# qradiolink/qradiolink

Measured on AMD Instinct MI355X. Metric: IQ MSamples/sec through RX demod chain, higher is better.
Workload: dtype f32

## Files before the change

### include/qrl_hip.h

```cpp
#ifndef QRL_HIP_H
#define QRL_HIP_H
#include <stddef.h>
#include <stdint.h>

#ifdef __cplusplus
extern "C" {
#endif

typedef enum {
    QRL_OK = 0,
    QRL_ERR_ARG = -1,
    QRL_ERR_NO_DEVICE = -2,
    QRL_ERR_HIP = -3,
    QRL_ERR_NOMEM = -4,
    QRL_ERR_TOO_BIG = -5,
    QRL_ERR_STATE = -6
} qrl_status;

enum {
    QRL_MODEM_BPSK2K = 0, QRL_MODEM_QPSK20K = 1, QRL_MODEM_QPSKVIDEO = 2, QRL_MODEM_4FSK2K = 3, QRL_MODEM_4FSK10KFM = 4, QRL_MODEM_4FSK2KFM = 5, QRL_MODEM_4FSK1KFM = 6, QRL_MODEM_QPSK2K = 7,
    QRL_MODEM_NBFM2500 = 8, QRL_MODEM_NBFM5000 = 9, QRL_MODEM_WBFM = 10, QRL_MODEM_USB2500 = 11, QRL_MODEM_LSB2500 = 12, QRL_MODEM_CW600USB = 13 , QRL_MODEM_AM5000 = 14,
    QRL_MODEM_2FSK2KFM = 15, QRL_MODEM_2FSK1KFM = 16, QRL_MODEM_2FSK2K = 17, QRL_MODEM_2FSK1K = 18,
    QRL_MODEM_2FSK10KFM = 19, QRL_MODEM_GMSK2K = 20, QRL_MODEM_GMSK1K = 21, QRL_MODEM_GMSK10K = 22,
    QRL_MODEM_BPSK1K = 24, QRL_MODEM_BPSK8 = 25 , QRL_MODEM_QPSK250K = 26, QRL_MODEM_4FSK100K = 27, QRL_MODEM_M17 = 40, QRL_MODEM_DMR = 41
// ... 18 lines not shown
    size_t max_chunk;
    void* hip_stream;
    int enable_side_outputs;
    int time_domain_samp_rate;
    double time_domain_filter_width;
} qrl_demod_config;

typedef struct {
    float* filtered;      size_t filtered_cap;
    float* constellation; size_t constellation_cap;
    uint8_t* bits_a;      size_t bits_cap;
    uint8_t* bits_b;
    uint32_t* counts;
    float* audio;         size_t audio_cap;
} qrl_demod_out;

int qrl_demod_create(qrl_ctx* ctx, const qrl_demod_config* cfg, qrl_demod** out);
void qrl_demod_destroy(qrl_demod* d);
int qrl_demod_reset(qrl_demod* d);
int qrl_demod_set_carrier_offset(qrl_demod* d, double carrier_offset_hz);
int qrl_demod_set_carrier_offsets(qrl_demod* d, const double* hz);
#define QRL_DMO_RECORD_BYTES 40
int qrl_demod_set_dmo_output(qrl_demod* d, uint8_t* frames, size_t cap_frames, uint32_t* counts);
enum { QRL_OPT_OVERLAP = 1, QRL_OPT_UNFUSED_DEC2 = 2, QRL_OPT_FLL_SLIM = 3 , QRL_OPT_GROUPED = 4, QRL_OPT_INPUT_RESIDENT = 5 };
int qrl_demod_set_option(qrl_demod* d, int option, int value);
int qrl_demod_out_caps(const qrl_demod* d, size_t n, size_t* filtered_cap, size_t* constellation_cap, size_t* bits_cap);
int qrl_demod_audio_cap(const qrl_demod* d, size_t n, size_t* audio_cap);
int qrl_demod_set_squelch(qrl_demod* d, double db);
int qrl_demod_time_domain_cap(const qrl_demod* d, size_t n, size_t* cap);
int qrl_demod_set_time_domain_output(qrl_demod* d, float* samples, size_t cap, uint32_t* counts);
int qrl_demod_set_ctcss(qrl_demod* d, float tone_hz);
int qrl_demod_set_agc(qrl_demod* d, float attack, float decay);
int qrl_demod_set_filter_width(qrl_demod* d, int filter_width);
int qrl_demod_set_gain(qrl_demod* d, float value);

int qrl_demod_process(qrl_demod* d, const float* iq, size_t stride, size_t n, const qrl_demod_out* out);
int qrl_demod_sync(qrl_demod* d);
void* qrl_demod_stream(qrl_demod* d);
int qrl_demod_internal_streams(qrl_demod* d, void* out[3]);
int qrl_demod_stream_wait(qrl_demod* d, void* hip_stream);

int qrl_demod_profile(qrl_demod* d, int enable);
int qrl_demod_profile_read(qrl_demod* d, double* kernel_ms, uint64_t* launches, const char** kernel_name);

int qrl_demod_process_host(qrl_demod* d, const float* iq_host, size_t stride, size_t n,
                           uint8_t* bits_a_host, uint8_t* bits_b_host, size_t bits_cap, uint32_t* counts_host);

// ... 170 lines not shown
```

### qradiolink_amd/__init__.py

```python
import ctypes as C
import os

import numpy as np

_HERE = os.path.dirname(os.path.abspath(__file__))
LIB_PATH = os.environ.get("QRL_LIB_PATH") or os.path.join(_HERE, "libqrl_hip.so")

MODEM_2FSK2KFM, MODEM_2FSK1KFM, MODEM_2FSK2K, MODEM_2FSK1K, MODEM_2FSK10KFM = 15, 16, 17, 18, 19
MODEM_GMSK2K, MODEM_GMSK1K, MODEM_GMSK10K = 20, 21, 22
MODEM_QPSK250K = 26
MODEM_QPSK20K, MODEM_QPSKVIDEO, MODEM_QPSK2K = 1, 2, 7
MODEM_BPSK2K, MODEM_BPSK1K = 0, 24
MODEM_4FSK2K, MODEM_4FSK10KFM, MODEM_4FSK2KFM, MODEM_4FSK1KFM, MODEM_4FSK100K = 3, 4, 5, 6, 27
MODEM_BPSK8 = 25
MODEM_NBFM2500, MODEM_NBFM5000, MODEM_WBFM, MODEM_AM5000 = 8, 9, 10, 14
MODEM_USB2500, MODEM_LSB2500, MODEM_CW600USB = 11, 12, 13
MODEM_M17 = 40
MODEM_DMR = 41
OPT_OVERLAP, OPT_UNFUSED_DEC2, OPT_FLL_SLIM, OPT_GROUPED, OPT_INPUT_RESIDENT = 1, 2, 3, 4, 5
CHAN_OPT_LEGACY_PFB, CHAN_OPT_LEGACY_TAIL, CHAN_OPT_SERIAL_TAIL = 1, 2, 3
WIN_HAMMING, WIN_HANN, WIN_BLACKMAN, WIN_RECTANGULAR, WIN_BLACKMAN_HARRIS = 0, 1, 2, 3, 5


class QrlError(RuntimeError):
    pass


class _Config(C.Structure):
    _fields_ = [("modem_type", C.c_int), ("use_mode_defaults", C.c_int), ("sps", C.c_int), ("samp_rate", C.c_int),
                ("carrier_freq", C.c_int), ("filter_width", C.c_int), ("fm", C.c_int), ("device_samp_rate", C.c_int),
                ("carrier_offset_hz", C.c_double), ("batch", C.c_int), ("max_chunk", C.c_size_t),
                ("hip_stream", C.c_void_p), ("enable_side_outputs", C.c_int), ("time_domain_samp_rate", C.c_int), ("time_domain_filter_width", C.c_double)]


class _ModConfig(C.Structure):
    _fields_ = [("modem_type", C.c_int), ("use_mode_defaults", C.c_int), ("sps", C.c_int), ("samp_rate", C.c_int),
                ("carrier_freq", C.c_int), ("filter_width", C.c_int), ("fm", C.c_int), ("batch", C.c_int),
                ("max_bytes", C.c_size_t), ("hip_stream", C.c_void_p), ("bb_gain", C.c_float),
                ("device_samp_rate", C.c_int), ("carrier_offset_hz", C.c_double)]


class _ChanConfig(C.Structure):
# ... 900 lines not shown
```

### qradiolink_amd/csrc/devmath.hpp

```cpp
#pragma once
#include <hip/hip_runtime.h>
#include <stdint.h>
#include "../../include/qrl_contracts.h"

namespace qrl {

__device__ __forceinline__ float poly_sin(float x)
{
    const float z = x * x;
    float p = fmaf(z, -1.9515295891e-4f, 8.3321608736e-3f);
    p = fmaf(z, p, -1.6666654611e-1f);
    return fmaf(x * z, p, x);
}
__device__ __forceinline__ float poly_cos(float x)
{
    const float z = x * x;
    float p = fmaf(z, 2.443315711809948e-5f, -1.388731625493765e-3f);
    p = fmaf(z, p, 4.166664568298827e-2f);
    const float q = fmaf(z, -0.5f, 1.0f);
    return fmaf(z * z, p, q);
}
__device__ __forceinline__ float2 quad_fix(int q, float ps, float pc)
{
    const bool swap = q & 1;
    const uint32_t c0 = __float_as_uint(swap ? ps : pc), s0 = __float_as_uint(swap ? pc : ps);
    const uint32_t negc = ((uint32_t)(q + 1) & 2u) << 30, negs = ((uint32_t)q & 2u) << 30;
    return make_float2(__uint_as_float(c0 ^ negc), __uint_as_float(s0 ^ negs));
}
// ... 103 lines not shown
```

### qradiolink_amd/csrc/engine.cpp

```cpp
#include "host_common.hpp"
#include "firdes.hpp"
#include <algorithm>
#include <cmath>
#include <complex>
#include <cstdio>
#include <cstdlib>
#include <cstring>
#include <memory>
#include <new>
#include <string>
#include <mutex>
#include <set>
#include <vector>

using namespace qrl;

static thread_local std::string g_last_error;
int qrl_set_error(int code, const std::string& msg) { g_last_error = msg; return code; }

namespace qrl {
static thread_local bool t_launch_error = false;
hipError_t dyn_lds_limit(const void* kernel, int bytes)
{
    static std::mutex mu;
// ... 177 lines not shown
    }
};

}

struct qrl_demod {
    qrl_ctx* ctx = nullptr;
    qrl_demod_config cfg{};
    hipStream_t stream = nullptr;
    bool own_stream = false;
    hipStream_t tail = nullptr;
    hipStream_t fecs = nullptr;
    hipEvent_t ev_q[2] = {nullptr, nullptr}, ev_fec[2] = {nullptr, nullptr}; bool q_valid[2] = {false, false};
    bool grouped = false, grouped_capable = false, fec_deferred = false; FecParams fec_pending{}; int fec_pending_slot = 0;
    DevBuf<uint64_t> qp_snap;
    hipEvent_t ev_ff = nullptr, ev_tail = nullptr;
    hipStream_t pre = nullptr; hipEvent_t ev_pre = nullptr, ev_fe[2] = {nullptr, nullptr}; bool fe_valid[2] = {false, false}; bool pre_pending = false;
    bool input_resident = false;
    hipEvent_t ev_user[4] = {nullptr, nullptr, nullptr, nullptr};
    bool tail_pending = false;
    bool qpsk_fll = false, fsk4_disc = false;
    bool m17 = false;
    DevBuf<float2> s2g, disc4_taps; DevBuf<float> sym4_taps; int disc4_nt = 0, sym4_nt = 0;
    bool fll_slim = false;
    bool d2f_capable = false, d2f = false; DevBuf<float> d2f_taps;
    bool overlap = false, overlap_capable = false; hipEvent_t ev_tail2[2] = {nullptr, nullptr}; bool tail2_valid[2] = {false, false}; uint64_t call_no = 0;
    enum Family { F_2FSK, F_GMSK, F_QPSK, F_DMR, F_4FSK, F_BPSK, F_DSSS, F_ANALOG } fam = F_2FSK;
    int branches = 2;

    int fe_decim = 1, interp = 1, decim = 1, target = 0, sps_eff = 0;
    bool fm = false;

    DecimStage fe;
    DecimStage first;
    DecimStage scope; DevBuf<float2> s_scope; uint32_t scope_mask = 0; uint64_t n_scope = 0; int scope_D = 10;
    float2* scope_out = nullptr; size_t scope_cap = 0; uint32_t* scope_counts = nullptr;
    DevBuf<float> rs_taps; int rs_Jp = 0;
    DevBuf<float> filt_taps; int filt_nt = 0;
    DevBuf<float> symf_taps; int symf_nt = 0;
    DevBuf<float2> disc_up, disc_lo; int disc_nt = 0;
    DevBuf<float> ff_tf, ff_ts; DevBuf<float2> ff_up, ff_lo;
    DevBuf<float2> fll_lo, fll_up; float fll_alpha = 0, fll_beta = 0, fll_maxf = 0;
    DevBuf<float> atan_tab, mmse_tab;
    float demod_gain = 0;
    float ss_alpha = 0, ss_beta = 0, ss_maxp = 0, ss_minp = 0;

// ... 535 lines not shown
        if (use_pre) {
            if (fe_valid[slot ^ 1]) HIPCHK(hipStreamWaitEvent(pre, ev_fe[slot ^ 1], 0));
            launch_hist_save(h, B, pre);
            HIPCHK(hipEventRecord(ev_pre, pre));
            pre_pending = true;
        } else launch_hist_save(h, B, stream);
        hist_flip = !hist_flip;
    }
    if (overlap) {
        HIPCHK(hipEventRecord(ev_ff, stream));
        HIPCHK(hipStreamWaitEvent(tail, ev_ff, 0));
        HIPCHK(hipMemsetAsync(counts, 0, (size_t)B * 4 * sizeof(uint32_t), tail));
    }
    const uint32_t c2 = (uint32_t)(n2_1 - n2_0);
    const bool side = cfg.enable_side_outputs && out;
    if (fam == F_DSSS || fam == F_ANALOG) {
        if (int rr = fam == F_DSSS ? dsss_stages(n2_0, n2_1, out, counts, side) : analog_stages(n2_0, n2_1, out, counts, side)) return rr;
        HIPCHK(hipGetLastError());
        if (take_launch_error()) return QRL_ERR_HIP;
        n_in = n_in1; n1 = n1_1; n2 = n2_1; ++call_no;
        return QRL_OK;
    }
    RingC filt_in = r2;
    if (fam == F_2FSK || fam == F_BPSK || (fam == F_QPSK && qpsk_fll)) {
        FllParams f{};
        f.in = r2; f.out = r2l; f.q0 = n2_0; f.count = c2; f.st = fll_st.p;
        f.lower = fll_lo.p; f.upper = fll_up.p; f.nt = fam == F_2FSK ? 16 : 32; f.alpha = fll_alpha; f.beta = fll_beta; f.max_freq = fll_maxf;
        f.slim = fll_slim ? 1 : 0;
        if (!(QRL_DEV_SKIP & 1)) launch_fll(f, B, cs);
        filt_in = r2l;
    }
    const bool fused_2fsk = fam == F_2FSK && !fm && filt_nt <= 41 && disc_nt <= 41 && symf_nt <= 25;
    if (fam == F_DMR) {
        RingC dem_in = r2;
        if (m17) {
            FirCcfParams f{};
            f.in = r2; f.out = r2f; f.q0 = n2_0; f.count = c2; f.taps = filt_taps.p; f.nt = filt_nt;
            f.port = side && out->filtered ? reinterpret_cast<float2*>(out->filtered) : nullptr;
            f.port_cap = side ? out->filtered_cap : 0;
            f.counts = counts;
            launch_fir_ccf(f, B, cs);
            dem_in = r2f;
        }
        QuadDemodParams q{}; q.in = dem_in; q.out = r2d; q.q0 = n2_0; q.count = c2; q.gain = demod_gain; q.atan_tab = atan_tab.p;
        launch_quad_demod(q, B, cs);
        if (!overlap && tail_pending) { HIPCHK(hipStreamWaitEvent(stream, ev_tail, 0)); tail_pending = false; }
        FirFffParams f{}; f.in = r2d; f.out = r3; f.q0 = n2_0; f.count = c2; f.taps = symf_taps.p; f.nt = symf_nt;
        launch_fir_fff(f, B, cs);
        if (!overlap) { HIPCHK(hipEventRecord(ev_ff, stream)); HIPCHK(hipStreamWaitEvent(tail, ev_ff, 0)); }
    } else if (fused_2fsk) {
        if (!overlap && tail_pending) { HIPCHK(hipStreamWaitEvent(stream, ev_tail, 0)); tail_pending = false; }
        Fsk2FfParams f{};
        f.in = filt_in; f.out = r3; f.q0 = n2_0; f.count = c2;
        f.tf = ff_tf.p; f.nf = fsk2_ff_padded(filt_nt); f.up = ff_up.p; f.lo = ff_lo.p; f.nb = fsk2_ff_padded(disc_nt);
        f.ts = ff_ts.p; f.ns = fsk2_ff_padded(symf_nt);
        f.port = side && out->filtered ? reinterpret_cast<float2*>(out->filtered) : nullptr;
        f.port_cap = side ? out->filtered_cap : 0;
        f.counts = counts;
        if (!(QRL_DEV_SKIP & 2)) launch_2fsk_ff(f, B, cs);
        if (!overlap) { HIPCHK(hipEventRecord(ev_ff, stream)); HIPCHK(hipStreamWaitEvent(tail, ev_ff, 0)); }
    } else {
        if (!d2f) {
            FirCcfParams f{};
            f.in = filt_in; f.out = r2f; f.q0 = n2_0; f.count = c2; f.taps = filt_taps.p; f.nt = filt_nt;
            f.port = side && out->filtered ? reinterpret_cast<float2*>(out->filtered) : nullptr;
            f.port_cap = side ? out->filtered_cap : 0;
            f.counts = counts;
            launch_fir_ccf(f, B, cs);
        }
        if (fam == F_QPSK || fam == F_BPSK) {
        } else if (fsk4_disc) {
            RingC r2l4{s2l.p, s2_mask}, r2g{s2g.p, s2_mask};
            Disc4fskParams d{}; d.in = r2f; d.out = r2l4; d.q0 = n2_0; d.count = c2; d.taps = disc4_taps.p; d.nt = disc4_nt;
            launch_disc_4fsk(d, B, cs);
            FirCcfParams f{}; f.in = r2l4; f.out = r2g; f.q0 = n2_0; f.count = c2; f.taps = sym4_taps.p; f.nt = sym4_nt;
            launch_fir_ccf(f, B, cs);
        } else if (fam == F_GMSK || fam == F_4FSK || fm) {
            QuadDemodParams q{}; q.in = r2f; q.out = r2d; q.q0 = n2_0; q.count = c2; q.gain = demod_gain; q.atan_tab = atan_tab.p;
            launch_quad_demod(q, B, cs);
        } else {
            Disc2fskParams d{}; d.in = r2f; d.out = r2d; d.q0 = n2_0; d.count = c2; d.up = disc_up.p; d.lo = disc_lo.p; d.nt = disc_nt;
            launch_disc_2fsk(d, B, cs);
// ... 383 lines not shown
        if (int rs = d->sync_all()) return rs;
        if ((r = d->dmo_st.alloc(d->cfg.batch)) || (r = d->dmo_golay.upload(golay1987_table()))) return r;
        std::vector<DmoState> ds(d->cfg.batch);
        for (auto& x : ds) { std::memset(&x, 0, sizeof x); x.endPtr = 9999; }
        if (hipMemcpy(d->dmo_st.p, ds.data(), ds.size() * sizeof(DmoState), hipMemcpyHostToDevice) != hipSuccess) return QRL_ERR_HIP;
    }
    d->dmo_out = frames; d->dmo_cap = (uint32_t)cap_frames; d->dmo_counts = counts;
    return QRL_OK;
}
int qrl_demod_set_option(qrl_demod* d, int option, int value)
{
    if (!d) return QRL_ERR_ARG;
    switch (option) {
    case QRL_OPT_OVERLAP:
        if (value != 0 && !d->overlap_capable) return qrl_set_error(QRL_ERR_ARG, "overlapped mode exists for the 2FSK family only");
        if (int rs = d->sync_all()) return rs;
        d->overlap = value != 0;
        d->tail2_valid[0] = d->tail2_valid[1] = false;
        return QRL_OK;
    case QRL_OPT_FLL_SLIM:
        if (int rs = d->sync_all()) return rs;
        d->fll_slim = value != 0;
        return QRL_OK;
    case QRL_OPT_GROUPED:
        if (value != 0 && !d->grouped_capable) return qrl_set_error(QRL_ERR_ARG, "the grouped order exists for the gr_demod_qpsk chain only");
        if (int rs = d->sync_all()) return rs;
        d->grouped = value != 0;
        return QRL_OK;
    case QRL_OPT_INPUT_RESIDENT: {
        if (int rs = d->sync_all()) return rs;
        if (value != 0 && d->pre) {
            DecimStage& st = d->fe.used ? d->fe : d->first;
            if (st.edge_len && !st.edge_b.p) if (int r = st.edge_b.alloc((size_t)d->cfg.batch * st.edge_len)) return qrl_set_error(r, "edge scratch");
        }
        d->input_resident = value != 0;
        return QRL_OK;
    }
    case QRL_OPT_UNFUSED_DEC2:
        if (!d->d2f_capable) return qrl_set_error(QRL_ERR_ARG, "this chain has no fused 1:2 decimator + shaping filter");
        if (d->n_in != 0) return qrl_set_error(QRL_ERR_STATE, "QRL_OPT_UNFUSED_DEC2 can only be set before the first sample (the two forms carry different state)");
        d->d2f = value == 0;
        return QRL_OK;
    default:
        return qrl_set_error(QRL_ERR_ARG, "unknown option");
    }
}
// ... 221 lines not shown
```

### qradiolink_amd/csrc/engine.hpp

```cpp
#pragma once
#include <hip/hip_runtime.h>
#include <stdint.h>
#include <vector>

namespace qrl {

hipError_t dyn_lds_limit(const void* kernel, int bytes);
bool take_launch_error();

int create_role_stream(hipStream_t* s, int priority, const char* role);

struct RingC { float2* p; uint32_t mask; };
struct RingF { float* p; uint32_t mask; };
struct RingB { uint8_t* p; uint32_t mask; };

template <class Pp>
__device__ __forceinline__ void rot_select(Pp& c, const Pp& p, uint32_t b)
{
    c = p; c.rot_acc = p.rot_acc_s[b]; c.rot_inc = p.rot_inc_s[b]; c.rot_lo = p.rot_lo + (size_t)b * 512;
}
#define ROT_VIEW(T, PS, P, SRC, B) T P##_ps_; if constexpr (PS) rot_select(P##_ps_, SRC, (uint32_t)(B)); const T& P = (PS) ? P##_ps_ : SRC
std::vector<float2> rot_fine_table(uint64_t inc);
void launch_rot_ps_advance(uint64_t* acc, const uint64_t* inc, int B, uint64_t delta, hipStream_t s);
void launch_rot_ps_fill(uint64_t* acc, uint64_t* inc, float2* lo, int B, int set_acc, uint64_t acc0, uint64_t inc0, const float2* lo0, hipStream_t s);
// ... 72 lines not shown
                      float2* port; size_t port_cap; uint32_t* counts; };
struct FirFffParams { RingF in; RingF out; uint64_t q0; uint32_t count; const float* taps; int nt; };
struct QuadDemodParams { RingC in; RingF out; uint64_t q0; uint32_t count; float gain; const float* atan_tab;
                         RingF out2; float gain2;
                         int16_t* s16; size_t s16_cap; float s16_level, s16_scale; uint32_t* s16_counts; };
struct Disc2fskParams { RingC in; RingF out; uint64_t q0; uint32_t count; const float2* up; const float2* lo; int nt; };
struct Disc4fskParams { RingC in; RingC out; uint64_t q0; uint32_t count; const float2* taps; int nt; };
void launch_disc_4fsk(const Disc4fskParams& p, int batch, hipStream_t s);
struct Fsk2FfParams { RingC in; RingF out; uint64_t q0; uint32_t count;
                      const float* tf; int nf; const float2* up; const float2* lo; int nb; const float* ts; int ns;
                      float2* port; size_t port_cap; uint32_t* counts; };
void launch_2fsk_ff(const Fsk2FfParams& p, int batch, hipStream_t s);
int fsk2_ff_padded(int n);
void launch_fir_ccf(const FirCcfParams& p, int batch, hipStream_t s);
void launch_fir_fff(const FirFffParams& p, int batch, hipStream_t s);
void launch_quad_demod(const QuadDemodParams& p, int batch, hipStream_t s);
void launch_disc_2fsk(const Disc2fskParams& p, int batch, hipStream_t s);

struct FllState { float phase, freq; float2 dl[32]; };
struct FllParams { RingC in; RingC out; uint64_t q0; uint32_t count; FllState* st;
                   const float2* lower; const float2* upper; int nt; float alpha, beta, max_freq;
                   int slim; };
void launch_fll(const FllParams& p, int batch, hipStream_t s);

struct SymSyncState { uint64_t ii; uint64_t oo; float mu, avg, inst; float x0, x1, x2, d0, d1, d2; };
struct SymSyncParams {
    RingF in; uint64_t avail;
    RingB soft;
    SymSyncState* st;
    const float* mmse;
    float alpha, beta, maxp, minp;
    int ted; float soft_mul, soft_add;
    int slicer;
    float tail_scale;
    int tail;
    uint8_t* bits; size_t bits_cap;
    float2* port; size_t port_cap; uint32_t* counts;
    int slim;
};
void launch_symsync_ff(const SymSyncParams& p, int batch, hipStream_t s);

struct QpskState {
    uint64_t ii, oo;
    float gain;
    float c1_phase, c1_freq;
    float mu, avg, inst;
// ... 202 lines not shown
```

### qradiolink_amd/csrc/kernels_ff.hip

```cpp
#include "devmath.hpp"
#include "engine.hpp"
#include <cstdlib>

namespace qrl {

__device__ __forceinline__ float2 ringc_at(const RingC& r, int b, int64_t i)
{
    if (i < 0) return make_float2(0.f, 0.f);
    return r.p[(size_t)b * (r.mask + 1u) + ((uint32_t)i & r.mask)];
}
__device__ __forceinline__ float ringf_at(const RingF& r, int b, int64_t i)
{
    if (i < 0) return 0.f;
    return r.p[(size_t)b * (r.mask + 1u) + ((uint32_t)i & r.mask)];
}

__global__ __launch_bounds__(256) void k_fir_ccf(const FirCcfParams P)
{
    const int b = blockIdx.y;
    const uint32_t t = blockIdx.x * 256u + threadIdx.x;
    if (t >= P.count) return;
    if (t == 0 && P.counts) P.counts[b * 4 + 0] = P.count;
    const int64_t n = (int64_t)(P.q0 + t);
    float ar = 0.f, ai = 0.f;
// ... 172 lines not shown
    const float m3 = sqrtf(re[2] * re[2] + im[2] * im[2]), m4 = sqrtf(re[3] * re[3] + im[3] * im[3]);
    const float A = 0.707107f;
    float2 v = make_float2(0.f, 0.f);
    if (m1 > m2 && m1 > m3 && m1 > m4) v = make_float2(-A, -A);
    else if (m2 > m1 && m2 > m3 && m2 > m4) v = make_float2(-A, A);
    else if (m3 > m2 && m3 > m1 && m3 > m4) v = make_float2(A, A);
    else if (m4 > m2 && m4 > m1 && m4 > m3) v = make_float2(A, -A);
    P.out.p[(size_t)b * (P.out.mask + 1u) + ((uint32_t)n & P.out.mask)] = v;
}
void launch_disc_4fsk(const Disc4fskParams& p, int batch, hipStream_t s)
{
    if (!p.count) return;
    hipLaunchKernelGGL(k_disc_4fsk, dim3((p.count + 255) / 256, batch), dim3(256), 0, s, p);
}

void launch_disc_2fsk(const Disc2fskParams& p, int batch, hipStream_t s)
{
    if (!p.count) return;
    hipLaunchKernelGGL(k_disc_2fsk, dim3((p.count + 255) / 256, batch), dim3(256), 0, s, p);
}

constexpr int FF_PL = 280, FF_PF = 264, FF_PD = 264;

template <int PITCH, int NQ, typename TapT, typename ItemT, typename Fma>
__device__ __forceinline__ void ff_window4(const ItemT* __restrict__ tile, int w, int nq_rt, const TapT* __restrict__ taps, Fma&& fma4)
{
    ItemT cur[4], nxt[4];
#pragma unroll
    for (int s = 0; s < 4; ++s) cur[s] = tile[s * PITCH + w];
    auto quad = [&](int q) {
        --w;
#pragma unroll
        for (int s = 0; s < 4; ++s) nxt[s] = tile[s * PITCH + w];
        const TapT h0 = taps[4 * q], h1 = taps[4 * q + 1], h2 = taps[4 * q + 2], h3 = taps[4 * q + 3];
        fma4(h0, cur[0], cur[1], cur[2], cur[3]);
        fma4(h1, nxt[3], cur[0], cur[1], cur[2]);
        fma4(h2, nxt[2], nxt[3], cur[0], cur[1]);
        fma4(h3, nxt[1], nxt[2], nxt[3], cur[0]);
#pragma unroll
        for (int s = 0; s < 4; ++s) cur[s] = nxt[s];
    };
    if constexpr (NQ > 0) {
#pragma unroll 4
        for (int q = 0; q < NQ; ++q) quad(q);
    } else {
        for (int q = 0; q < nq_rt; ++q) quad(q);
    }
}

template <int NQF, int NQB, int NQS>
__global__ __launch_bounds__(256) void k_2fsk_ff(const Fsk2FfParams P)
{
    __shared__ float2 lt[4 * FF_PL];
    __shared__ float2 ft[4 * FF_PF];
    __shared__ float dt[4 * FF_PD];
    const int b = blockIdx.y, tid = threadIdx.x;
    const int hf = P.nf - 1, hb = P.nb - 1, hs = P.ns - 1;
    const int T = 1024 - hb - hs;
    const int64_t n0t = (int64_t)P.q0 + (int64_t)blockIdx.x * T;
    const int nl = 1024 + hf, nd = T + hs;
    if (tid < 4) { lt[tid * FF_PL] = make_float2(0.f, 0.f); ft[tid * FF_PF] = make_float2(0.f, 0.f); dt[tid * FF_PD] = 0.f; }
    {
        float2 v[5];
#pragma unroll
        for (int it = 0; it < 5; ++it) {
            const int64_t a = n0t - (hf + hb + hs) + tid + 256 * it;
            v[it] = P.in.p[(size_t)b * (P.in.mask + 1u) + ((uint32_t)a & P.in.mask)];
            if (a < 0) v[it] = make_float2(0.f, 0.f);
        }
#pragma unroll
        for (int it = 0; it < 5; ++it) {
            const int i = tid + 256 * it;
            if (i < nl) lt[(i & 3) * FF_PL + (i >> 2) + 1] = v[it];
        }
    }
    __syncthreads();
    {
        float2 a[4] = {{0.f, 0.f}, {0.f, 0.f}, {0.f, 0.f}, {0.f, 0.f}};
        ff_window4<FF_PL, NQF>(lt, tid + (hf >> 2) + 1, (hf >> 2) + 1, P.tf,
                          [&](float h, const float2& x0, const float2& x1, const float2& x2, const float2& x3) {
                              a[0].x = fmaf(h, x0.x, a[0].x); a[0].y = fmaf(h, x0.y, a[0].y);
                              a[1].x = fmaf(h, x1.x, a[1].x); a[1].y = fmaf(h, x1.y, a[1].y);
                              a[2].x = fmaf(h, x2.x, a[2].x); a[2].y = fmaf(h, x2.y, a[2].y);
                              a[3].x = fmaf(h, x3.x, a[3].x); a[3].y = fmaf(h, x3.y, a[3].y);
                          });
#pragma unroll
        for (int r = 0; r < 4; ++r) {
            const bool neg = n0t - (hb + hs) + 4 * tid + r < 0;
            ft[r * FF_PF + tid + 1] = neg ? make_float2(0.f, 0.f) : a[r];
        }
    }
    __syncthreads();
    if (4 * tid < nd) {
        float ar[4] = {0.f, 0.f, 0.f, 0.f}, ai[4] = {0.f, 0.f, 0.f, 0.f}, br[4] = {0.f, 0.f, 0.f, 0.f}, bi[4] = {0.f, 0.f, 0.f, 0.f};
        const int nq = NQB > 0 ? NQB : (hb >> 2) + 1;
        int w = tid + (hb >> 2) + 1;
        float2 cur[4], nxt[4];
#pragma unroll
        for (int s = 0; s < 4; ++s) cur[s] = ft[s * FF_PF + w];
        auto step = [&](const float2 h, const float2& x0, const float2& x1, const float2& x2, const float2& x3) {
// ... 13 lines not shown
            step(P.up[4 * q + 2], nxt[2], nxt[3], cur[0], cur[1]);
            step(P.up[4 * q + 3], nxt[1], nxt[2], nxt[3], cur[0]);
#pragma unroll
            for (int s = 0; s < 4; ++s) cur[s] = nxt[s];
        };
        if constexpr (NQB > 0) {
#pragma unroll 4
            for (int q = 0; q < NQB; ++q) quad(q);
        } else {
            for (int q = 0; q < nq; ++q) quad(q);
        }
#pragma unroll
        for (int r = 0; r < 4; ++r) {
            const float ur = ar[r] - bi[r], ui = ai[r] + br[r], lr = ar[r] + bi[r], li = ai[r] - br[r];
            const float mu = sqrtf(ur * ur + ui * ui);
            const float ml = sqrtf(lr * lr + li * li);
            float v = mu / ml;
            if (!(v >= 0.0f)) v = 0.0f;
            if (v > 2.0f) v = 2.0f;
            dt[r * FF_PD + tid + 1] = (n0t - hs + 4 * tid + r < 0) ? 0.f : v + (-1.0f);
        }
    }
    __syncthreads();
    if (4 * tid < T) {
        float a[4] = {0.f, 0.f, 0.f, 0.f};
        ff_window4<FF_PD, NQS>(dt, tid + (hs >> 2) + 1, (hs >> 2) + 1, P.ts,
                          [&](float h, float x0, float x1, float x2, float x3) {
                              a[0] = fmaf(h, x0, a[0]); a[1] = fmaf(h, x1, a[1]); a[2] = fmaf(h, x2, a[2]); a[3] = fmaf(h, x3, a[3]);
                          });
        const uint32_t t0 = blockIdx.x * (uint32_t)T + 4u * tid;
        if (t0 == 0 && P.counts) P.counts[b * 4 + 0] = P.count;
        const int wf = tid + ((hb + hs) >> 2) + 1;
#pragma unroll
        for (int r = 0; r < 4; ++r) {
            const uint32_t t = t0 + r;
            if (t < P.count) {
                const int64_t n = n0t + 4 * tid + r;
                P.out.p[(size_t)b * (P.out.mask + 1u) + ((uint32_t)n & P.out.mask)] = a[r];
                if (P.port && t < P.port_cap) P.port[(size_t)b * P.port_cap + t] = ft[r * FF_PF + wf];
            }
        }
    }
}
int fsk2_ff_padded(int n) { return (n - 1 + 3) / 4 * 4 + 1; }
void launch_2fsk_ff(const Fsk2FfParams& p, int batch, hipStream_t s)
{
    if (!p.count) return;
// ... 10 lines not shown
```

### qradiolink_amd/csrc/kernels_loops.hip

```cpp
#include "devmath.hpp"
#include "engine.hpp"

namespace qrl {


#ifndef QRL_FLL_CH
#define QRL_FLL_CH 32
#endif
#ifndef QRL_FLL_TH
#define QRL_FLL_TH 256
#endif
template <int CTRL> __device__ __forceinline__ float dpp_quad(float v)
{
    return __builtin_bit_cast(float, __builtin_amdgcn_mov_dpp(__builtin_bit_cast(int, v), CTRL, 0xF, 0xF, true));
}

template <int NT, int FLL_TH, int FLL_CH>
__global__ __launch_bounds__(FLL_TH) void k_fll(const FllParams P, int batch)
{
    constexpr int FLL_NS = FLL_TH / 4;
    constexpr int GL = NT / 4;
    __shared__ float2 win[FLL_NS][FLL_CH + 1];
    __shared__ float2 tl[NT], tu[NT];
    __shared__ float2 dump[FLL_TH];
    const int tid = threadIdx.x;
    const int sl = tid >> 2, g = tid & 3;
    const int b0 = blockIdx.x * FLL_NS;
    const int b = b0 + sl;
    const bool active = b < batch;
    for (int k = tid; k < NT; k += FLL_TH) { tl[k] = P.lower[k]; tu[k] = P.upper[k]; }
    float phase = 0.f, freq = 0.f;
    float2 dl[GL];
    if (active) {
        const FllState& s = P.st[b];
        phase = s.phase; freq = s.freq;
#pragma unroll
        for (int t = 0; t < GL; ++t) dl[t] = s.dl[g * GL + t];
    } else {
// ... 358 lines not shown
```

Baseline: 531,300.

## Fuse 2FSK FLL loop with feed-forward filter chain in one warp-specialized kernel

Adds a kernel where one set of wavefronts runs the serial FLL band-edge loop per stream while other wavefronts run the 2FSK FIR/discriminator/symbol-filter chain on the previous window, with the default option turning it on. This avoids the separate FLL kernel writing its output to a global ring and the FF kernel reading it back, and overlaps the latency-bound serial loop with the filter arithmetic. The standalone FF kernel also skips work past the valid count in the last block. The fused path adds prologue recomputation of lookahead windows and extra LDS, and it may lower occupancy.

Measured after the change: 507,400. -4.5%, worse.

```diff
diff --git a/include/qrl_hip.h b/include/qrl_hip.h
--- a/include/qrl_hip.h
+++ b/include/qrl_hip.h
@@ -64,7 +64,8 @@
 int qrl_demod_set_carrier_offsets(qrl_demod* d, const double* hz);
 #define QRL_DMO_RECORD_BYTES 40
 int qrl_demod_set_dmo_output(qrl_demod* d, uint8_t* frames, size_t cap_frames, uint32_t* counts);
-enum { QRL_OPT_OVERLAP = 1, QRL_OPT_UNFUSED_DEC2 = 2, QRL_OPT_FLL_SLIM = 3 , QRL_OPT_GROUPED = 4, QRL_OPT_INPUT_RESIDENT = 5 };
+enum { QRL_OPT_OVERLAP = 1, QRL_OPT_UNFUSED_DEC2 = 2, QRL_OPT_FLL_SLIM = 3 , QRL_OPT_GROUPED = 4, QRL_OPT_INPUT_RESIDENT = 5,
+       QRL_OPT_FUSED_FLL_FF = 6  };
 int qrl_demod_set_option(qrl_demod* d, int option, int value);
 int qrl_demod_out_caps(const qrl_demod* d, size_t n, size_t* filtered_cap, size_t* constellation_cap, size_t* bits_cap);
 int qrl_demod_audio_cap(const qrl_demod* d, size_t n, size_t* audio_cap);
diff --git a/qradiolink_amd/__init__.py b/qradiolink_amd/__init__.py
--- a/qradiolink_amd/__init__.py
+++ b/qradiolink_amd/__init__.py
@@ -17,7 +17,7 @@
 MODEM_USB2500, MODEM_LSB2500, MODEM_CW600USB = 11, 12, 13
 MODEM_M17 = 40
 MODEM_DMR = 41
-OPT_OVERLAP, OPT_UNFUSED_DEC2, OPT_FLL_SLIM, OPT_GROUPED, OPT_INPUT_RESIDENT = 1, 2, 3, 4, 5
+OPT_OVERLAP, OPT_UNFUSED_DEC2, OPT_FLL_SLIM, OPT_GROUPED, OPT_INPUT_RESIDENT, OPT_FUSED_FLL_FF = 1, 2, 3, 4, 5, 6
 CHAN_OPT_LEGACY_PFB, CHAN_OPT_LEGACY_TAIL, CHAN_OPT_SERIAL_TAIL = 1, 2, 3
 WIN_HAMMING, WIN_HANN, WIN_BLACKMAN, WIN_RECTANGULAR, WIN_BLACKMAN_HARRIS = 0, 1, 2, 3, 5
 
diff --git a/qradiolink_amd/csrc/devmath.hpp b/qradiolink_amd/csrc/devmath.hpp
--- a/qradiolink_amd/csrc/devmath.hpp
+++ b/qradiolink_amd/csrc/devmath.hpp
@@ -4,6 +4,11 @@
 #include "../../include/qrl_contracts.h"
 
 namespace qrl {
+
+template <int CTRL> __device__ __forceinline__ float dpp_quad(float v)
+{
+    return __builtin_bit_cast(float, __builtin_amdgcn_mov_dpp(__builtin_bit_cast(int, v), CTRL, 0xF, 0xF, true));
+}
 
 __device__ __forceinline__ float poly_sin(float x)
 {
diff --git a/qradiolink_amd/csrc/engine.cpp b/qradiolink_amd/csrc/engine.cpp
--- a/qradiolink_amd/csrc/engine.cpp
+++ b/qradiolink_amd/csrc/engine.cpp
@@ -223,6 +223,7 @@
     bool qpsk_fll = false, fsk4_disc = false;
     bool m17 = false;
     DevBuf<float2> s2g, disc4_taps; DevBuf<float> sym4_taps; int disc4_nt = 0, sym4_nt = 0;
+    int fused_fll_ff = 1;
     bool fll_slim = false;
     bool d2f_capable = false, d2f = false; DevBuf<float> d2f_taps;
     bool overlap = false, overlap_capable = false; hipEvent_t ev_tail2[2] = {nullptr, nullptr}; bool tail2_valid[2] = {false, false}; uint64_t call_no = 0;
@@ -804,15 +805,19 @@
         return QRL_OK;
     }
     RingC filt_in = r2;
+    const bool fused_2fsk = fam == F_2FSK && !fm && filt_nt <= 41 && disc_nt <= 41 && symf_nt <= 25;
+    FllFfParams fl{};
+    bool fused_fll = false;
     if (fam == F_2FSK || fam == F_BPSK || (fam == F_QPSK && qpsk_fll)) {
         FllParams f{};
         f.in = r2; f.out = r2l; f.q0 = n2_0; f.count = c2; f.st = fll_st.p;
         f.lower = fll_lo.p; f.upper = fll_up.p; f.nt = fam == F_2FSK ? 16 : 32; f.alpha = fll_alpha; f.beta = fll_beta; f.max_freq = fll_maxf;
         f.slim = fll_slim ? 1 : 0;
-        if (!(QRL_DEV_SKIP & 1)) launch_fll(f, B, cs);
+        fl.fll = f; fl.ff.nf = fsk2_ff_padded(filt_nt); fl.ff.nb = fsk2_ff_padded(disc_nt); fl.ff.ns = fsk2_ff_padded(symf_nt);
+        fused_fll = fused_2fsk && fused_fll_ff != 0 && fll_2fsk_supported(fl);
+        if (!fused_fll && !(QRL_DEV_SKIP & 1)) launch_fll(f, B, cs);
         filt_in = r2l;
     }
-    const bool fused_2fsk = fam == F_2FSK && !fm && filt_nt <= 41 && disc_nt <= 41 && symf_nt <= 25;
     if (fam == F_DMR) {
         RingC dem_in = r2;
         if (m17) {
@@ -839,7 +844,10 @@
         f.port = side && out->filtered ? reinterpret_cast<float2*>(out->filtered) : nullptr;
         f.port_cap = side ? out->filtered_cap : 0;
         f.counts = counts;
-        if (!(QRL_DEV_SKIP & 2)) launch_2fsk_ff(f, B, cs);
+        if (fused_fll) {
+            fl.ff = f; fl.geo = fused_fll_ff;
+            if (!(QRL_DEV_SKIP & 3)) launch_fll_2fsk(fl, B, cs);
+        } else if (!(QRL_DEV_SKIP & 2)) launch_2fsk_ff(f, B, cs);
         if (!overlap) { HIPCHK(hipEventRecord(ev_ff, stream)); HIPCHK(hipStreamWaitEvent(tail, ev_ff, 0)); }
     } else {
         if (!d2f) {
@@ -1269,6 +1277,11 @@
         if (int rs = d->sync_all()) return rs;
         d->fll_slim = value != 0;
         return QRL_OK;
+    case QRL_OPT_FUSED_FLL_FF:
+        if (value < 0 || value > 4) return qrl_set_error(QRL_ERR_ARG, "QRL_OPT_FUSED_FLL_FF: 0 (off), 1 (default geometry) .. 4");
+        if (int rs = d->sync_all()) return rs;
+        d->fused_fll_ff = value;
+        return QRL_OK;
     case QRL_OPT_GROUPED:
         if (value != 0 && !d->grouped_capable) return qrl_set_error(QRL_ERR_ARG, "the grouped order exists for the gr_demod_qpsk chain only");
         if (int rs = d->sync_all()) return rs;
diff --git a/qradiolink_amd/csrc/engine.hpp b/qradiolink_amd/csrc/engine.hpp
--- a/qradiolink_amd/csrc/engine.hpp
+++ b/qradiolink_amd/csrc/engine.hpp
@@ -118,6 +118,9 @@
                    const float2* lower; const float2* upper; int nt; float alpha, beta, max_freq;
                    int slim; };
 void launch_fll(const FllParams& p, int batch, hipStream_t s);
+struct FllFfParams { FllParams fll; Fsk2FfParams ff; int geo; };
+bool fll_2fsk_supported(const FllFfParams& p);
+void launch_fll_2fsk(const FllFfParams& p, int batch, hipStream_t s);
 
 struct SymSyncState { uint64_t ii; uint64_t oo; float mu, avg, inst; float x0, x1, x2, d0, d1, d2; };
 struct SymSyncParams {
diff --git a/qradiolink_amd/csrc/ff_window.hpp b/qradiolink_amd/csrc/ff_window.hpp
--- /dev/null
+++ b/qradiolink_amd/csrc/ff_window.hpp
@@ -0,0 +1,32 @@
+#pragma once
+#include <hip/hip_runtime.h>
+
+namespace qrl {
+
+template <int PITCH, int NQ, typename TapT, typename ItemT, typename Fma>
+__device__ __forceinline__ void ff_window4(const ItemT* __restrict__ tile, int w, int nq_rt, const TapT* __restrict__ taps, Fma&& fma4)
+{
+    ItemT cur[4], nxt[4];
+#pragma unroll
+    for (int s = 0; s < 4; ++s) cur[s] = tile[s * PITCH + w];
+    auto quad = [&](int q) {
+        --w;
+#pragma unroll
+        for (int s = 0; s < 4; ++s) nxt[s] = tile[s * PITCH + w];
+        const TapT h0 = taps[4 * q], h1 = taps[4 * q + 1], h2 = taps[4 * q + 2], h3 = taps[4 * q + 3];
+        fma4(h0, cur[0], cur[1], cur[2], cur[3]);
+        fma4(h1, nxt[3], cur[0], cur[1], cur[2]);
+        fma4(h2, nxt[2], nxt[3], cur[0], cur[1]);
+        fma4(h3, nxt[1], nxt[2], nxt[3], cur[0]);
+#pragma unroll
+        for (int s = 0; s < 4; ++s) cur[s] = nxt[s];
+    };
+    if constexpr (NQ > 0) {
+#pragma unroll 4
+        for (int q = 0; q < NQ; ++q) quad(q);
+    } else {
+        for (int q = 0; q < nq_rt; ++q) quad(q);
+    }
+}
+
+}
diff --git a/qradiolink_amd/csrc/kernels_ff.hip b/qradiolink_amd/csrc/kernels_ff.hip
--- a/qradiolink_amd/csrc/kernels_ff.hip
+++ b/qradiolink_amd/csrc/kernels_ff.hip
@@ -1,5 +1,6 @@
 #include "devmath.hpp"
 #include "engine.hpp"
+#include "ff_window.hpp"
 #include <cstdlib>
 
 namespace qrl {
@@ -218,32 +219,6 @@
 
 constexpr int FF_PL = 280, FF_PF = 264, FF_PD = 264;
 
-template <int PITCH, int NQ, typename TapT, typename ItemT, typename Fma>
-__device__ __forceinline__ void ff_window4(const ItemT* __restrict__ tile, int w, int nq_rt, const TapT* __restrict__ taps, Fma&& fma4)
-{
-    ItemT cur[4], nxt[4];
-#pragma unroll
-    for (int s = 0; s < 4; ++s) cur[s] = tile[s * PITCH + w];
-    auto quad = [&](int q) {
-        --w;
-#pragma unroll
-        for (int s = 0; s < 4; ++s) nxt[s] = tile[s * PITCH + w];
-        const TapT h0 = taps[4 * q], h1 = taps[4 * q + 1], h2 = taps[4 * q + 2], h3 = taps[4 * q + 3];
-        fma4(h0, cur[0], cur[1], cur[2], cur[3]);
-        fma4(h1, nxt[3], cur[0], cur[1], cur[2]);
-        fma4(h2, nxt[2], nxt[3], cur[0], cur[1]);
-        fma4(h3, nxt[1], nxt[2], nxt[3], cur[0]);
-#pragma unroll
-        for (int s = 0; s < 4; ++s) cur[s] = nxt[s];
-    };
-    if constexpr (NQ > 0) {
-#pragma unroll 4
-        for (int q = 0; q < NQ; ++q) quad(q);
-    } else {
-        for (int q = 0; q < nq_rt; ++q) quad(q);
-    }
-}
-
 template <int NQF, int NQB, int NQS>
 __global__ __launch_bounds__(256) void k_2fsk_ff(const Fsk2FfParams P)
 {
@@ -254,7 +229,8 @@
     const int hf = P.nf - 1, hb = P.nb - 1, hs = P.ns - 1;
     const int T = 1024 - hb - hs;
     const int64_t n0t = (int64_t)P.q0 + (int64_t)blockIdx.x * T;
-    const int nl = 1024 + hf, nd = T + hs;
+    const int need = (int)min((uint32_t)T, P.count - blockIdx.x * (uint32_t)T);
+    const int nl = 1024 + hf, nd = need + hs, nf1 = need + hs + hb;
     if (tid < 4) { lt[tid * FF_PL] = make_float2(0.f, 0.f); ft[tid * FF_PF] = make_float2(0.f, 0.f); dt[tid * FF_PD] = 0.f; }
     {
         float2 v[5];
@@ -271,7 +247,7 @@
         }
     }
     __syncthreads();
-    {
+    if (4 * tid < nf1) {
         float2 a[4] = {{0.f, 0.f}, {0.f, 0.f}, {0.f, 0.f}, {0.f, 0.f}};
         ff_window4<FF_PL, NQF>(lt, tid + (hf >> 2) + 1, (hf >> 2) + 1, P.tf,
                           [&](float h, const float2& x0, const float2& x1, const float2& x2, const float2& x3) {
@@ -331,7 +307,7 @@
         }
     }
     __syncthreads();
-    if (4 * tid < T) {
+    if (4 * tid < need) {
         float a[4] = {0.f, 0.f, 0.f, 0.f};
         ff_window4<FF_PD, NQS>(dt, tid + (hs >> 2) + 1, (hs >> 2) + 1, P.ts,
                           [&](float h, float x0, float x1, float x2, float x3) {
diff --git a/qradiolink_amd/csrc/kernels_fll_ff.hip b/qradiolink_amd/csrc/kernels_fll_ff.hip
--- /dev/null
+++ b/qradiolink_amd/csrc/kernels_fll_ff.hip
@@ -0,0 +1,297 @@
+#include "devmath.hpp"
+#include "engine.hpp"
+#include "ff_window.hpp"
+
+namespace qrl {
+
+namespace {
+__device__ __forceinline__ void wave_sync()
+{
+    __builtin_amdgcn_fence(__ATOMIC_RELEASE, "wavefront");
+    __builtin_amdgcn_wave_barrier();
+    __builtin_amdgcn_fence(__ATOMIC_ACQUIRE, "wavefront");
+}
+}
+
+template <int NS, int W> struct FllFfGeo {
+    static constexpr size_t lds_bytes() { return (size_t)NS * ((W + 1) * 8 + 2 * (44 + W) * 8 + (28 + W) * 4 + 4 * 8) + 2 * 16 * 8; }
+};
+
+template <int NS, int W>
+__global__ __launch_bounds__(NS * 8) void k_fll_2fsk(const FllFfParams P, int batch)
+{
+    constexpr int NT = 16, GL = NT / 4;
+    constexpr int NREC = NS * 4;
+    constexpr int HF = 40, HB = 40, HS = 24;
+    constexpr int HC = HF + 4, HD = HS + 4;
+    constexpr int PC = (HC + W) / 4, PD = (HD + W) / 4;
+    constexpr int LPS = W / 4;
+    constexpr int SPP = 64 / LPS;
+    constexpr int NPASS = 16 / SPP;
+    constexpr int LOOK = HF + HB + HS;
+    constexpr int NPRE = (LOOK + W - 1) / W;
+    static_assert(HF == HB, "the y and f tiles share their geometry");
+    extern __shared__ __align__(16) unsigned char fllff_smem[];
+    float2 (*win)[W + 1] = reinterpret_cast<float2 (*)[W + 1]>(fllff_smem);
+    float2 (*yt)[4 * PC] = reinterpret_cast<float2 (*)[4 * PC]>(&win[NS][0]);
+    float2 (*ft)[4 * PC] = yt + NS;
+    float2* tl = &ft[NS][0];
+    float2* tu = tl + NT;
+    float2* dump = tu + NT;
+    float (*dt)[4 * PD] = reinterpret_cast<float (*)[4 * PD]>(dump + NREC);
+    const int tid = threadIdx.x;
+    const bool rec = tid < NREC;
+    const int b0 = blockIdx.x * NS;
+    const int nstreams = min(NS, batch - b0);
+    const uint32_t count = P.fll.count;
+    const int nwin = (int)((count + W - 1) / W);
+    const RingC ry = P.fll.out;
+    for (int k = tid; k < NT; k += NS * 8) { tl[k] = P.fll.lower[k]; tu[k] = P.fll.upper[k]; }
+    __syncthreads();
+
+    const int sl = tid >> 2, g = tid & 3;
+    const bool active = rec && b0 + sl < batch;
+    float phase = 0.f, freq = 0.f;
+    float2 dl[GL], hu[GL], hl[GL];
+    constexpr int NPT = 16 * W / 64;
+    float2 pre[NPT];
+    const int lane = tid & 63, wv = (tid & (NREC - 1)) >> 6;
+    auto preload = [&](uint32_t c0) {
+#pragma unroll
+        for (int i = 0; i < NPT; ++i) {
+            const int idx = lane + 64 * i, s = min(16 * wv + idx / W, nstreams - 1), k = idx % W;
+            const int64_t a = (int64_t)(P.fll.q0 + c0 + k) - NT;
+            const float2 v = P.fll.in.p[(size_t)(b0 + s) * (P.fll.in.mask + 1u) + ((uint32_t)a & P.fll.in.mask)];
+            pre[i] = a >= 0 ? v : make_float2(0.f, 0.f);
+        }
+    };
+    if (rec) {
+#pragma unroll
+        for (int t = 0; t < GL; ++t) { dl[t] = make_float2(0.f, 0.f); hu[t] = tu[g * GL + t]; hl[t] = tl[g * GL + t]; }
+        if (active) {
+            const FllState& s = P.fll.st[b0 + sl];
+            phase = s.phase; freq = s.freq;
+#pragma unroll
+            for (int t = 0; t < GL; ++t) dl[t] = s.dl[g * GL + t];
+        }
+        preload(0);
+    }
+
+    const int ft_ = tid - NREC;
+    const int fs0 = 16 * (ft_ >> 6) + (ft_ & 63) / LPS, t = (ft_ & 63) % LPS;
+    const int64_t q0 = (int64_t)P.fll.q0;
+    const Fsk2FfParams& F = P.ff;
+    auto fir_window = [&](int64_t n0w) {
+#pragma unroll 1
+        for (int p = 0; p < NPASS; ++p) {
+            const int s = fs0 + p * SPP, b = b0 + s;
+            const bool live = b < batch;
+            const int64_t n = n0w + 4 * t;
+            {
+                float2 a[4] = {{0.f, 0.f}, {0.f, 0.f}, {0.f, 0.f}, {0.f, 0.f}};
+                ff_window4<PC, 11>(&yt[s][0], HC / 4 + t, 11, F.tf,
+                                   [&](float h, const float2& x0, const float2& x1, const float2& x2, const float2& x3) {
+                                       a[0].x = fmaf(h, x0.x, a[0].x); a[0].y = fmaf(h, x0.y, a[0].y);
+                                       a[1].x = fmaf(h, x1.x, a[1].x); a[1].y = fmaf(h, x1.y, a[1].y);
+                                       a[2].x = fmaf(h, x2.x, a[2].x); a[2].y = fmaf(h, x2.y, a[2].y);
+                                       a[3].x = fmaf(h, x3.x, a[3].x); a[3].y = fmaf(h, x3.y, a[3].y);
+                                   });
+#pragma unroll
+                for (int r = 0; r < 4; ++r) {
+                    const float2 v = n + r < 0 ? make_float2(0.f, 0.f) : a[r];
+                    ft[s][r * PC + HC / 4 + t] = v;
+                    const int64_t k = n + r - q0;
+                    if (live && F.port && k >= 0 && k < (int64_t)count && (uint64_t)k < F.port_cap) F.port[(size_t)b * F.port_cap + (size_t)k] = v;
+                }
+            }
+            wave_sync();
+            {
+                float ar[4] = {0.f, 0.f, 0.f, 0.f}, ai[4] = {0.f, 0.f, 0.f, 0.f}, br[4] = {0.f, 0.f, 0.f, 0.f}, bi[4] = {0.f, 0.f, 0.f, 0.f};
+                ff_window4<PC, 11>(&ft[s][0], HC / 4 + t, 11, F.up,
+                                   [&](const float2 h, const float2& x0, const float2& x1, const float2& x2, const float2& x3) {
+                                       const float2 xs[4] = {x0, x1, x2, x3};
+#pragma unroll
+                                       for (int r = 0; r < 4; ++r) {
+                                           ar[r] = fmaf(h.x, xs[r].x, ar[r]); ai[r] = fmaf(h.x, xs[r].y, ai[r]);
+                                           br[r] = fmaf(h.y, xs[r].x, br[r]); bi[r] = fmaf(h.y, xs[r].y, bi[r]);
+                                       }
+                                   });
+#pragma unroll
+                for (int r = 0; r < 4; ++r) {
+                    const float ur = ar[r] - bi[r], ui = ai[r] + br[r], lr = ar[r] + bi[r], li = ai[r] - br[r];
+                    const float mu = sqrtf(ur * ur + ui * ui);
+                    const float ml = sqrtf(lr * lr + li * li);
+                    float v = mu / ml;
+                    if (!(v >= 0.0f)) v = 0.0f;
+                    if (v > 2.0f) v = 2.0f;
+                    dt[s][r * PD + HD / 4 + t] = n + r < 0 ? 0.f : v + (-1.0f);
+                }
+            }
+            wave_sync();
+            {
+                float a[4] = {0.f, 0.f, 0.f, 0.f};
+                ff_window4<PD, 7>(&dt[s][0], HD / 4 + t, 7, F.ts,
+                                  [&](float h, float x0, float x1, float x2, float x3) {
+                                      a[0] = fmaf(h, x0, a[0]); a[1] = fmaf(h, x1, a[1]); a[2] = fmaf(h, x2, a[2]); a[3] = fmaf(h, x3, a[3]);
+                                  });
+#pragma unroll
+                for (int r = 0; r < 4; ++r) {
+                    const int64_t k = n + r - q0;
+                    if (live && k >= 0 && k < (int64_t)count) F.out.p[(size_t)b * (F.out.mask + 1u) + ((uint32_t)(n + r) & F.out.mask)] = a[r];
+                }
+            }
+            {
+                constexpr int NC = (HC + LPS - 1) / LPS, ND = (HD + LPS - 1) / LPS;
+                float2 vy[NC], vf[NC];
+                float vd[ND];
+#pragma unroll
+                for (int i = 0; i < NC; ++i) {
+                    const int e = min(t + LPS * i, HC - 1), o = (e & 3) * PC + (e >> 2) + W / 4;
+                    vy[i] = yt[s][o]; vf[i] = ft[s][o];
+                }
+#pragma unroll
+                for (int i = 0; i < ND; ++i) {
+                    const int e = min(t + LPS * i, HD - 1);
+                    vd[i] = dt[s][(e & 3) * PD + (e >> 2) + W / 4];
+                }
+                wave_sync();
+#pragma unroll
+                for (int i = 0; i < NC; ++i) {
+                    const int e = t + LPS * i, o = (e & 3) * PC + (e >> 2);
+                    if (e < HC) { yt[s][o] = vy[i]; ft[s][o] = vf[i]; }
+                }
+#pragma unroll
+                for (int i = 0; i < ND; ++i) {
+                    const int e = t + LPS * i;
+                    if (e < HD) dt[s][(e & 3) * PD + (e >> 2)] = vd[i];
+                }
+            }
+            wave_sync();
+        }
+    };
+    if (!rec) {
+        for (int p = 0; p < NPASS; ++p) {
+            const int s = fs0 + p * SPP;
+            for (int i = t; i < 4 * PC; i += LPS) { yt[s][i] = make_float2(0.f, 0.f); ft[s][i] = make_float2(0.f, 0.f); }
+            for (int i = t; i < 4 * PD; i += LPS) dt[s][i] = 0.f;
+        }
+        wave_sync();
+#pragma unroll 1
+        for (int w = 0; w < NPRE; ++w) {
+            const int64_t n0w = q0 - (int64_t)(NPRE - w) * W;
+            for (int p = 0; p < NPASS; ++p) {
+                const int s = fs0 + p * SPP, bb = min(b0 + s, batch - 1);
+#pragma unroll
+                for (int r = 0; r < 4; ++r) {
+                    const int64_t a = n0w + 4 * t + r;
+                    float2 v = ry.p[(size_t)bb * (ry.mask + 1u) + ((uint32_t)a & ry.mask)];
+                    if (a < 0 || a < q0 - LOOK) v = make_float2(0.f, 0.f);
+                    yt[s][r * PC + HC / 4 + t] = v;
+                }
+            }
+            wave_sync();
+            fir_window(n0w);
+        }
+    }
+
+    for (int c = 0; c < nwin; ++c) {
+        const uint32_t c0 = (uint32_t)c * W;
+        const int len = min((uint32_t)W, count - c0);
+        if (rec) {
+#pragma unroll
+            for (int i = 0; i < NPT; ++i) { const int idx = lane + 64 * i; win[16 * wv + idx / W][idx % W] = pre[i]; }
+            wave_sync();
+            if (c + 1 < nwin) preload(c0 + W);
+            if (active) {
+                for (int k = 0; k < len; ++k) {
+                    const float2 x = win[sl][k];
+                    const float2 nco = sincos_rad(phase);
+                    float2 carry;
+                    carry.x = dpp_quad<0x90>(dl[GL - 1].x);
+                    carry.y = dpp_quad<0x90>(dl[GL - 1].y);
+#pragma unroll
+                    for (int t2 = GL - 1; t2 > 0; --t2) dl[t2] = dl[t2 - 1];
+                    float ur = 0.f, ui = 0.f, lr = 0.f, li = 0.f;
+#pragma unroll
+                    for (int t2 = GL - 1; t2 >= 1; --t2) {
+                        const float2 v = dl[t2];
+                        ur = fmaf(hu[t2].x, v.x, ur); ur = fmaf(-hu[t2].y, v.y, ur);
+                        ui = fmaf(hu[t2].x, v.y, ui); ui = fmaf(hu[t2].y, v.x, ui);
+                        lr = fmaf(hl[t2].x, v.x, lr); lr = fmaf(-hl[t2].y, v.y, lr);
+                        li = fmaf(hl[t2].x, v.y, li); li = fmaf(hl[t2].y, v.x, li);
+                    }
+                    const float2 y = cmul(x, nco);
+                    *(g == 0 ? &win[sl][k] : &dump[tid]) = y;
+                    dl[0] = g == 0 ? y : carry;
+                    {
+                        const float2 v = dl[0];
+                        ur = fmaf(hu[0].x, v.x, ur); ur = fmaf(-hu[0].y, v.y, ur);
+                        ui = fmaf(hu[0].x, v.y, ui); ui = fmaf(hu[0].y, v.x, ui);
+                        lr = fmaf(hl[0].x, v.x, lr); lr = fmaf(-hl[0].y, v.y, lr);
+                        li = fmaf(hl[0].x, v.y, li); li = fmaf(hl[0].y, v.x, li);
+                    }
+                    ur = ur + dpp_quad<0xB1>(ur); ui = ui + dpp_quad<0xB1>(ui); lr = lr + dpp_quad<0xB1>(lr); li = li + dpp_quad<0xB1>(li);
+                    ur = ur + dpp_quad<0x4E>(ur); ui = ui + dpp_quad<0x4E>(ui); lr = lr + dpp_quad<0x4E>(lr); li = li + dpp_quad<0x4E>(li);
+                    const float error = (lr * lr + li * li) - (ur * ur + ui * ui);
+                    freq = freq + P.fll.beta * error;
+                    phase = phase + freq + P.fll.alpha * error;
+                    phase = phase_wrap(phase);
+                    freq = __builtin_fminf(__builtin_fmaxf(freq, -P.fll.max_freq), P.fll.max_freq);
+                }
+            }
+        } else if (c > 0) {
+            fir_window(q0 + (int64_t)(c0 - W));
+        }
+        __syncthreads();
+        if (!rec) {
+            for (int p = 0; p < NPASS; ++p) {
+                const int s = fs0 + p * SPP, b = b0 + s;
+#pragma unroll
+                for (int r = 0; r < 4; ++r) {
+                    const uint32_t k = c0 + 4 * t + r;
+                    const float2 v = win[s][4 * t + r];
+                    yt[s][r * PC + HC / 4 + t] = v;
+                    if (b < batch && k < count && k + LOOK >= count)
+                        ry.p[(size_t)b * (ry.mask + 1u) + ((uint32_t)(P.fll.q0 + k) & ry.mask)] = v;
+                }
+            }
+        }
+        __syncthreads();
+    }
+    if (!rec) {
+        fir_window(q0 + (int64_t)(nwin - 1) * W);
+        if (t == 0 && F.counts)
+            for (int p = 0; p < NPASS; ++p) { const int b = b0 + fs0 + p * SPP; if (b < batch) F.counts[b * 4 + 0] = count; }
+    } else if (active) {
+        FllState& s = P.fll.st[b0 + sl];
+        if (g == 0) { s.phase = phase; s.freq = freq; }
+#pragma unroll
+        for (int t2 = 0; t2 < GL; ++t2) s.dl[g * GL + t2] = dl[t2];
+    }
+}
+
+bool fll_2fsk_supported(const FllFfParams& p)
+{
+    return p.fll.nt == 16 && p.ff.nf == 41 && p.ff.nb == 41 && p.ff.ns == 25;
+}
+
+template <int NS, int W> static void launch_geo(const FllFfParams& p, int batch, hipStream_t s)
+{
+    const auto k = k_fll_2fsk<NS, W>;
+    const size_t lds = FllFfGeo<NS, W>::lds_bytes();
+    if (dyn_lds_limit(reinterpret_cast<const void*>(k), (int)lds) != hipSuccess) return;
+    hipLaunchKernelGGL(k, dim3((batch + NS - 1) / NS), dim3(NS * 8), lds, s, p, batch);
+}
+
+void launch_fll_2fsk(const FllFfParams& p, int batch, hipStream_t s)
+{
+    if (!p.fll.count) return;
+    switch (p.geo) {
+    case 2: launch_geo<64, 32>(p, batch, s); break;
+    case 3: launch_geo<16, 16>(p, batch, s); break;
+    case 4: launch_geo<64, 16>(p, batch, s); break;
+    default: launch_geo<16, 32>(p, batch, s); break;
+    }
+}
+
+}
diff --git a/qradiolink_amd/csrc/kernels_loops.hip b/qradiolink_amd/csrc/kernels_loops.hip
--- a/qradiolink_amd/csrc/kernels_loops.hip
+++ b/qradiolink_amd/csrc/kernels_loops.hip
@@ -10,10 +10,6 @@
 #ifndef QRL_FLL_TH
 #define QRL_FLL_TH 256
 #endif
-template <int CTRL> __device__ __forceinline__ float dpp_quad(float v)
-{
-    return __builtin_bit_cast(float, __builtin_amdgcn_mov_dpp(__builtin_bit_cast(int, v), CTRL, 0xF, 0xF, true));
-}
 
 template <int NT, int FLL_TH, int FLL_CH>
 __global__ __launch_bounds__(FLL_TH) void k_fll(const FllParams P, int batch)
```
